# tj12323/GeoPurify

Hardware: AMD Instinct MI355X
Metric: scenes/sec (ScanNet-val shape) + pooled-feature GB/s vs HBM peak (higher is better)
Workload: dtype f32 (student convolutions and pooling: f16 hi/lo split operands, 3 MFMAs per product, fp32 accumulate)

## Files before the change

geopurify_amd/_lib.py:

```python
import ctypes
import os
from ctypes import POINTER, c_char_p, c_double, c_float, c_int32, c_int64, c_size_t, c_uint32, c_uint64, c_void_p

_HERE = os.path.dirname(os.path.abspath(__file__))
LIB_PATH = os.environ.get("GP_LIB") or os.path.join(_HERE, "libgeopurify_hip.so")

_P = c_void_p
GP_KNN_MAX_K = 127
GP_KNN_QUERY_MAX_K = 32
GP_ELEM_F32, GP_ELEM_F16, GP_ELEM_BF16 = 0, 1, 2
GP_LABEL_U8, GP_LABEL_I16, GP_LABEL_I32, GP_LABEL_I64 = 0, 1, 2, 3

SIGNATURES = {
    "gp_version": (c_int32, []),
    "gp_last_error": (c_char_p, []),
    "gp_debug_set": (c_int32, [c_int32, c_int32]),
    "gp_debug_ptr": (c_int32, [c_int32, _P, c_size_t]),
    "gp_voxelize_workspace_bytes": (c_size_t, [c_int64]),
    "gp_voxelize_f64": (c_int32, [_P, c_int64, POINTER(c_double), _P, _P, _P, _P, _P, _P, _P, c_size_t, _P]),
    "gp_fnv_hash_f64": (c_int32, [_P, c_int64, _P, _P]),
    "gp_project_points_f64": (c_int32, [_P, c_int64, POINTER(c_double), c_double, c_double, c_double,
                                        c_double, _P, c_int32, c_int32, c_int32, c_double, _P, _P, _P]),
    "gp_render_depth_f64": (c_int32, [_P, c_int64, POINTER(c_double), c_double, c_double, c_double, c_double,
                                      c_int32, c_int32, c_int32, _P, _P]),
# ... 11 lines not shown
    "gp_quantize_batched_workspace_bytes": (c_size_t, [c_int64]),
    "gp_quantize_batched": (c_int32, [_P, c_int64, _P, _P, _P, _P, _P, _P, _P, c_size_t, _P]),
    "gp_segment_labels": (c_int32, [_P, c_int64, _P, _P, _P, c_int64, c_int64, c_int32, _P, _P]),
    "gp_sparse_conv": (c_int32, [_P, c_int64, _P, c_int64, _P, c_int32, c_int32, c_int32, _P, _P, _P,
                                 c_int64, c_int32, _P, c_int64, _P]),
    "gp_conv_pairs_workspace_bytes": (c_size_t, [c_int64, c_int32]),
    "gp_conv_pairs_build": (c_int32, [_P, c_int64, c_int32, c_int32, _P, _P, _P, _P, _P, _P, _P, c_size_t, _P]),
    "gp_conv_chunk_plan_workspace_bytes": (c_size_t, [c_int64, c_int32]),
    "gp_conv_chunk_plan": (c_int32, [_P, c_int64, c_int32, c_int32, c_int32, c_int32, c_int32, _P, _P, _P, c_size_t, _P]),
    "gp_conv_weights_split": (c_int32, [_P, c_int32, c_int32, c_int32, c_float, _P, _P, _P]),
    "gp_split_f16": (c_int32, [_P, c_int64, c_int32, c_int64, _P, _P, c_int64, _P]),
    "gp_sparse_conv_f16x3": (c_int32, [_P, c_int64, _P, _P, c_int64, _P, _P, _P, _P, _P, c_int32, c_int64, c_int64, c_int32, _P, _P,
                                       c_int32, c_int32, _P, _P, _P, _P, c_int64, c_int32, _P, c_int64, _P, _P,
                                       c_int64, c_int32, POINTER(c_int32), POINTER(c_int32), POINTER(c_int32), _P, _P,
                                       _P, _P, c_int64, _P, c_int32, c_int32, _P]),
    "gp_conv_weights_split_blocked": (c_int32, [_P, c_int32, c_int32, c_int32, c_float, _P, _P, c_int32, _P]),
    "gp_pow2_scale": (c_int32, [_P, c_int64, c_int32, c_int64, _P, _P, c_size_t, _P]),
    "gp_voxel_rows_operands": (c_int32, [_P, c_int64, c_int32, _P, c_int64, c_int32, _P, _P, c_int64, _P, _P, c_int64, c_int32, _P, c_int64,
                                         _P, _P, _P, c_size_t, _P]),
    "gp_split_f16_scaled": (c_int32, [_P, c_int64, c_int32, c_int64, _P, _P, c_int64, _P, _P, _P, _P]),
    "gp_rcb_order": (c_int32, [_P, c_int64, c_int32, c_int32, _P, _P, _P]),
    "gp_rows_renumber_i32": (c_int32, [_P, c_int64, c_int32, _P, _P, _P, _P]),
    "gp_l2norm_rows": (c_int32, [_P, c_int64, c_int32, c_int64, _P]),
    "gp_embed_head_f16x3": (c_int32, [_P, _P, c_int64, _P, _P, _P, c_int64, c_int32, c_int32, c_float, c_int32, _P, c_int64, _P, _P, c_float, _P, _P]),
    "gp_knn_workspace_bytes": (c_size_t, [c_int64]),
    "gp_knn_lattice": (c_int32, [_P, _P, _P, c_int64, c_int32, _P, _P, c_size_t, _P]),
    "gp_knn_lattice_two_pass": (c_int32, [_P, _P, _P, c_int64, c_int32, _P, _P, c_size_t, _P]),
    "gp_knn_batched_workspace_bytes": (c_size_t, [c_int64]),
    "gp_knn_batched": (c_int32, [_P, _P, c_int64, c_int32, _P, _P, _P, c_size_t, _P]),
    "gp_affinity_softmax": (c_int32, [_P, c_int64, c_int32, _P, c_int32, c_int64, c_float, _P, _P]),
# ... 232 lines not shown
```

geopurify_amd/csrc/sparse_conv_v2.hip:

```cpp
#include <cstring>
#include <type_traits>
#include <rocprim/device/device_scan.hpp>

#include <hip/hip_fp16.h>

#include <stdlib.h>

#include "gp_common.h"
#include "gp_gfx950.h"
#include "gp_scan_bytes.h"

namespace {

constexpr int TM = 256, TN = 256, TK = 32;
constexpr int NT2 = 512;
constexpr int APITCH = 32;
__device__ __forceinline__ int sw_slot(int row, int slot) {
    const int h = (0x78 >> (((row >> 2) & 3) * 2)) & 3;
    return slot ^ h;
}

__device__ __forceinline__ void pair_decode(int64_t i, int kv, const int32_t *__restrict__ R, int nchunks, int &c, int &k, int64_t &u) {
    const int row_q = (int)(i / kv);
    int lo = 0, hi = nchunks - 1;
// ... 22 lines not shown
__global__ void pair_emit_kernel(const int32_t *__restrict__ nm, const int32_t *__restrict__ sc, int64_t nv, int kv,
                                 const int32_t *__restrict__ R, int nchunks, int32_t *__restrict__ pair_in, int32_t *__restrict__ pair_pos,
                                 int32_t *__restrict__ seg_off ) {
    int64_t total = (int64_t)kv * nv;
    int64_t i = blockIdx.x * (int64_t)blockDim.x + threadIdx.x;
    if (i >= total) return;
    int c, k; int64_t u;
    pair_decode(i, kv, R, nchunks, c, k, u);
    u = u < 0 ? 0 : (u >= nv ? nv - 1 : u);
    int in = nm[(int64_t)k * nv + u];
    int s = sc[i];
    pair_pos[(int64_t)k * nv + u] = in >= 0 ? s : -1;
    if (in >= 0) pair_in[s] = in;
    if (u == (int64_t)R[c]) seg_off[c * kv + k] = s;
    if (i == total - 1) seg_off[(c + 1) * kv] = s + (in >= 0 ? 1 : 0);
}
__global__ void chunk_count_kernel(const int32_t *__restrict__ nm, int64_t nv, int kv, int granule, int32_t *__restrict__ cnt ) {
    const int g = blockIdx.x, k = blockIdx.y;
    const int64_t r0 = (int64_t)g * granule, r1 = r0 + granule < nv ? r0 + granule : nv;
    int c = 0;
    for (int64_t u = r0 + threadIdx.x; u < r1; u += blockDim.x) c += nm[(int64_t)k * nv + u] >= 0;
    c = gp_wave_sum(c);
    __shared__ int s_c[4];
    if (gp_lane() == 0) s_c[threadIdx.x >> 6] = c;
    __syncthreads();
    if (threadIdx.x == 0) cnt[g * 32 + k] = s_c[0] + s_c[1] + s_c[2] + s_c[3];
}
constexpr int CP_WIN = 512;
__device__ __forceinline__ int cp_sum32(int v) {
    v += __builtin_amdgcn_update_dpp(0, v, 0xB1, 0xF, 0xF, true);
// ... 735 lines not shown
__device__ __forceinline__ void q24_batch_decode(const u32x4 (&th)[NL], const u32x2 (&tl)[NL], const unsigned (&te)[NL], const unsigned (&tsel)[NL],
                                                 int cnt, unsigned q, bool act, float (&a)[8]) {
#pragma unroll
    for (int i = 0; i < NL; ++i)
        if (i < cnt && act) q24_row_decode(th[i], tl[i], __builtin_amdgcn_perm(0u, te[i], tsel[i] + q), a);
}

template <bool WIDE , bool NO_CENTRE = false ,
          int WALK = 0 >
__global__ void __launch_bounds__(256) __attribute__((amdgpu_waves_per_eu(WALK ? GP_P2_WAVES : 4, WALK ? GP_P2_WAVES : 4)))
conv_phase2_q24_kernel(const unsigned char *__restrict__ pb, int64_t e_off, const int32_t *__restrict__ pair_pos, int64_t nv,
                       int kv, int cout, const float *__restrict__ scale, const float *__restrict__ shift,
                       const float *__restrict__ residual, int64_t ld_res, int relu, float *__restrict__ y, int64_t ld_y,
                       _Float16 *__restrict__ y_hi, _Float16 *__restrict__ y_lo, int64_t ld_yh, int64_t row_begin, int64_t row_count,
                       int pair_base, float *__restrict__ y_inv_scale, const _Float16 *__restrict__ res_hi,
                       const _Float16 *__restrict__ res_lo, int64_t ld_rh, const float *__restrict__ res_inv, int plane_flags) {
    const bool y_il = (plane_flags & 2) != 0, r_il = (plane_flags & 4) != 0;
    const int lane = gp_lane();
    const int64_t wave0 = (blockIdx.x * (int64_t)blockDim.x + threadIdx.x) >> 6, n_waves = ((int64_t)gridDim.x * blockDim.x) >> 6;
    const int64_t row_end = (row_begin + row_count < nv) ? row_begin + row_count : nv;
    int64_t u = row_begin + wave0;
    if (u >= row_end) return;
    const bool rowscale = y_inv_scale && y_hi && cout <= 1024;
    const int kv_read = NO_CENTRE ? (kv >> 1) : -1;
    int mypos_next = (lane < kv && lane != kv_read) ? pair_pos[(int64_t)lane * nv + u] : -1;
    float sc0[8], sh0[8];
    {
        const int c = lane * 8;
#pragma unroll
        for (int h = 0; h < 2; ++h) {
            const float4 a = (scale && c < cout) ? *reinterpret_cast<const float4 *>(scale + c + h * 4) : make_float4(1.f, 1.f, 1.f, 1.f);
            const float4 b = (shift && c < cout) ? *reinterpret_cast<const float4 *>(shift + c + h * 4) : make_float4(0.f, 0.f, 0.f, 0.f);
            sc0[h * 4] = a.x; sc0[h * 4 + 1] = a.y; sc0[h * 4 + 2] = a.z; sc0[h * 4 + 3] = a.w;
            sh0[h * 4] = b.x; sh0[h * 4 + 1] = b.y; sh0[h * 4 + 2] = b.z; sh0[h * 4 + 3] = b.w;
        }
    }
    if constexpr (WALK != 0) {
        static_assert(!WIDE && !NO_CENTRE, "the pipelined walk is for cout = 256 and 512");
        constexpr int NQ = 2 * WALK, NL = GP_P2_NL;
        const int c = lane * 8;
        const bool act = c < NQ * 128;
        const unsigned q = (unsigned)c >> 7, f = ((unsigned)c >> 3) & 15u;
        const unsigned off16 = q * 384u + f * 16u, off8 = q * 384u + 256u + f * 8u;
        const unsigned char *pb_e = pb + e_off;
        const unsigned long long kvmask = (kv >= 64) ? ~0ull : ((1ull << kv) - 1ull);
        auto load_pos = [&](int64_t r) { return (lane < kv && r < row_end) ? pair_pos[(int64_t)lane * nv + r] : -1; };
        auto wait_all = [] { __builtin_amdgcn_s_waitcnt(0x0f70); };
        u32x4 thA[NL], thB[NL];
        u32x2 tlA[NL], tlB[NL];
        unsigned teA[NL], teB[NL], tselA[NL], tselB[NL];
        int cntA, cntB;
        int posA = mypos_next, posB = load_pos(u + n_waves);
        unsigned long long mA = __ballot(posA >= 0) & kvmask;
        q24_batch_issue<NL, NQ>(thA, tlA, teA, tselA, cntA, pb, pb_e, posA, mA, off16, off8, act, pair_base);
        wait_all();
        unsigned long long mB = __ballot(posB >= 0) & kvmask;
        q24_batch_issue<NL, NQ>(thB, tlB, teB, tselB, cntB, pb, pb_e, posB, mB, off16, off8, act, pair_base);
        int pos2 = load_pos(u + 2 * n_waves);
        auto row = [&](u32x4 (&th)[NL], u32x2 (&tl)[NL], unsigned (&te)[NL], unsigned (&tsel)[NL], int &cnt, int &posX, unsigned long long &mX) __attribute__((always_inline)) {
            u32x4 r0 = {0u, 0u, 0u, 0u}, r1 = {0u, 0u, 0u, 0u};
            float ri = 1.f;
            if (act) {
                if (residual) {
                    r0 = *reinterpret_cast<const u32x4 *>(residual + u * ld_res + c);
                    r1 = *reinterpret_cast<const u32x4 *>(residual + u * ld_res + c + 4);
                } else if (res_hi) {
                    const _Float16 *rph = r_il ? res_hi + u * ld_rh + ((c >> 5) << 6) + (c & 31) : res_hi + u * ld_rh + c;
                    const _Float16 *rpl = r_il ? rph + 32 : res_lo + u * ld_rh + c;
                    r0 = *reinterpret_cast<const u32x4 *>(rph);
                    r1 = *reinterpret_cast<const u32x4 *>(rpl);
                    if (res_inv) ri = res_inv[u];
                }
            }
            float a[8];
#pragma unroll
            for (int j = 0; j < 8; ++j) a[j] = 0.f;
            q24_batch_decode<NL>(th, tl, te, tsel, cnt, q, act, a);
            while (mX) {
                q24_batch_issue<NL, NQ>(th, tl, te, tsel, cnt, pb, pb_e, posX, mX, off16, off8, act, pair_base);
                q24_batch_decode<NL>(th, tl, te, tsel, cnt, q, act, a);
            }
            wait_all();
            float amax = 0.f;
// ... 2 lines not shown
                for (int j = 0; j < 8; ++j) a[j] = a[j] * sc0[j] + sh0[j];
                if (residual) {
#pragma unroll
                    for (int j = 0; j < 4; ++j) { a[j] += __uint_as_float(r0[j]); a[j + 4] += __uint_as_float(r1[j]); }
                }
                if (res_hi) {
                    const f16x8 rh = __builtin_bit_cast(f16x8, r0), rl = __builtin_bit_cast(f16x8, r1);
#pragma unroll
                    for (int j = 0; j < 8; ++j) a[j] += ((float)rh[j] + (float)rl[j]) * ri;
                }
                if (relu) {
#pragma unroll
                    for (int j = 0; j < 8; ++j) a[j] = fmaxf(a[j], 0.f);
                }
                if (y) {
                    *reinterpret_cast<float4 *>(y + u * ld_y + c) = make_float4(a[0], a[1], a[2], a[3]);
                    *reinterpret_cast<float4 *>(y + u * ld_y + c + 4) = make_float4(a[4], a[5], a[6], a[7]);
                }
#pragma unroll
                for (int j = 0; j < 8; ++j) amax = fmaxf(amax, fabsf(a[j]));
            }
            float s = 1.f;
            if (rowscale) {
                amax = gp_wave_max(amax);
                s = gp_pow2_for(amax);
                if (lane == 0) y_inv_scale[u] = 1.f / s;
            }
            if (y_hi && act) {
                f16x8 h, l;
#pragma unroll
                for (int j = 0; j < 8; ++j) gp_split_f16(a[j] * s, h, l, j);
                _Float16 *ph = y_il ? y_hi + u * ld_yh + ((c >> 5) << 6) + (c & 31) : y_hi + u * ld_yh + c;
                _Float16 *pl = y_il ? ph + 32 : y_lo + u * ld_yh + c;
                *reinterpret_cast<f16x8 *>(ph) = h;
                *reinterpret_cast<f16x8 *>(pl) = l;
            }
            posX = pos2;
            mX = __ballot(posX >= 0) & kvmask;
            q24_batch_issue<NL, NQ>(th, tl, te, tsel, cnt, pb, pb_e, posX, mX, off16, off8, act, pair_base);
            pos2 = load_pos(u + 3 * n_waves);
        };
        for (;;) {
            row(thA, tlA, teA, tselA, cntA, posA, mA);
            u += n_waves;
            if (u >= row_end) break;
            row(thB, tlB, teB, tselB, cntB, posB, mB);
            u += n_waves;
            if (u >= row_end) break;
// ... 216 lines not shown
    size_t tb = gp_scan_bytes<int32_t>(total);
    char *tmp = cv.take<char>(tb);
    if (!cv.ok()) { gp_set_error("gp_conv_pairs_build: workspace too small (%zu < %zu)", workspace_bytes, cv.off); return GP_ENOMEM; }
    hipStream_t s = gp_stream(stream_);
    int blocks = (int)((total + 255) / 256);
    int nseg = num_chunks * kv;
    pair_flags_kernel<<<blocks, 256, 0, s>>>(nbr_map, nv, kv, chunk_row_off, num_chunks, f);
    GP_CHECK_HIP(rocprim::exclusive_scan(tmp, tb, f, sc, (int32_t)0, (size_t)total, rocprim::plus<int32_t>(), s));
    pair_emit_kernel<<<blocks, 256, 0, s>>>(nbr_map, sc, nv, kv, chunk_row_off, num_chunks, pair_in, pair_pos, seg_off);
    tile_start_kernel<<<1, 64, 0, s>>>(seg_off, nseg, tile_start);
    tile_desc_kernel<<<(nseg + 255) / 256, 256, 0, s>>>(seg_off, tile_start, nseg, kv, reinterpret_cast<int4 *>(tile_desc));
    GP_CHECK_LAUNCH();
    return GP_OK;
}

extern "C" size_t gp_conv_chunk_plan_workspace_bytes(int64_t nv, int32_t granule_rows) {
    if (nv <= 0 || granule_rows <= 0) return 0;
    return (size_t)((nv + granule_rows - 1) / granule_rows) * 32 * sizeof(int32_t);
}
extern "C" int gp_conv_chunk_plan(const int32_t *nbr_map, int64_t nv, int32_t kv, int32_t granule_rows, int32_t col_tiles,
                                  int32_t target_tiles, int32_t max_chunks, int32_t *chunk_row_off, int32_t *n_chunks, void *workspace,
                                  size_t workspace_bytes, void *stream_) {
    GP_CHECK_ARG(nbr_map && chunk_row_off && n_chunks && workspace && nv > 0 && kv > 0 && kv <= 32, "gp_conv_chunk_plan: null/empty argument");
    GP_CHECK_ARG(granule_rows >= 64 && granule_rows <= 65535 && col_tiles >= 1 && target_tiles >= col_tiles && max_chunks >= 1, "gp_conv_chunk_plan: bad sizes");
    const int64_t ngran = (nv + granule_rows - 1) / granule_rows;
    GP_CHECK_ARG(workspace_bytes >= gp_conv_chunk_plan_workspace_bytes(nv, granule_rows), "gp_conv_chunk_plan: workspace too small");
    hipStream_t s = gp_stream(stream_);
    int32_t *cnt = static_cast<int32_t *>(workspace);
    chunk_count_kernel<<<dim3((unsigned)ngran, (unsigned)kv), 256, 0, s>>>(nbr_map, nv, kv, granule_rows, cnt);
    chunk_plan_kernel<<<1, 256, 0, s>>>(cnt, (int)ngran, kv, granule_rows, nv, col_tiles, target_tiles, max_chunks, chunk_row_off, n_chunks);
// ... 41 lines not shown
    return GP_OK;
}

extern "C" int gp_split_f16_scaled(const float *x, int64_t ld_x, int32_t d, int64_t n, void *hi, void *lo, int64_t ld_h,
                                   const float *scale, float *row_inv_scale, const int32_t *dst_row, void *stream_) {
    GP_CHECK_ARG(x && hi && n > 0 && d > 0 && d % 4 == 0 && ld_x % 4 == 0 && ld_h % 4 == 0, "gp_split_f16_scaled: bad argument");
    GP_CHECK_ARG(lo || (d % 32 == 0 && ld_h >= 2 * (int64_t)d), "gp_split_f16_scaled: lo = NULL asks for interleaved rows in hi: d %% 32 == 0 and ld_h >= 2 d");
    GP_CHECK_ARG(!(scale && row_inv_scale), "gp_split_f16_scaled: one global scale OR per-row scales");
    int64_t waves = n < 16384 ? n : 16384;
    split_rows_scaled_kernel<<<(unsigned)((waves * 64 + 255) / 256), 256, 0, gp_stream(stream_)>>>(
        x, ld_x, d, n, static_cast<_Float16 *>(hi), static_cast<_Float16 *>(lo), ld_h, scale, row_inv_scale, dst_row);
    GP_CHECK_LAUNCH();
    return GP_OK;
}

extern "C" int gp_sparse_conv_f16x3(const float *x, int64_t ld_x, const void *x_hi, const void *x_lo, int64_t ld_xh,
                                    const int32_t *pair_in, const int32_t *pair_pos,
                                    const int32_t *pair_off, const int32_t *tile_start, const int32_t *tile_desc,
                                    int32_t nseg, int64_t num_pairs, int64_t nv, int32_t kv,
                                    const void *w_hi, const void *w_lo, int32_t cin, int32_t cout, float *partial,
                                    const float *scale, const float *shift, const float *residual, int64_t ld_res,
                                    int32_t relu, float *y, int64_t ld_y, void *y_hi, void *y_lo, int64_t ld_yh,
                                    int32_t num_chunks, const int32_t *chunk_row_off_host, const int32_t *chunk_tile_off_host,
                                    const int32_t *chunk_pair_off_host, const float *x_row_inv_scale, float *y_row_inv_scale,
                                    const void *res_hi, const void *res_lo, int64_t ld_rh, const float *res_row_inv_scale, int32_t w_blocked,
                                    int32_t plane_flags, void *stream_) {
    GP_CHECK_ARG(plane_flags >= 0 && plane_flags < 64, "gp_sparse_conv_f16x3: plane_flags is a mask of 1 (x interleaved), 2 (y interleaved), 4 (residual interleaved), 8 (fp32 partial rows), 16 (one dense offset: phase 1 writes y), 32 (phase 2 walks one row at a time)");
    const bool direct = (plane_flags & 16) != 0;
    GP_CHECK_ARG(!direct || (kv == 1 && num_pairs == nv && x_hi && y && ld_y == cout && !scale && !shift && !residual && !res_hi && !relu && !y_hi &&
                             !y_row_inv_scale && !(g_gp_knobs[3] & 16)),
                 "gp_sparse_conv_f16x3: plane_flags bit 4 is for kv = 1 with a pair for every row, pre-split x, contiguous fp32 y and no epilogue");
    GP_CHECK_ARG(!(plane_flags & 1) || (x_hi && ld_xh % 64 == 0 && cin % 32 == 0), "gp_sparse_conv_f16x3: interleaved x rows come as ONE tensor (x_hi) of 2 x cin halfs per row");
    GP_CHECK_ARG(!(plane_flags & 2) || (y_hi && ld_yh % 64 == 0 && (uintptr_t)y_hi % 16 == 0), "gp_sparse_conv_f16x3: interleaved y rows go to ONE tensor (y_hi) of 2 x cout halfs per row");
    GP_CHECK_ARG(!(plane_flags & 4) || (res_hi && ld_rh % 64 == 0), "gp_sparse_conv_f16x3: interleaved residual rows come as ONE tensor (res_hi)");
    GP_CHECK_ARG(w_blocked == 0 || w_blocked == 1, "gp_sparse_conv_f16x3: w_blocked is 0 (row-major weights) or 1 (gp_conv_weights_split_blocked)");
    GP_CHECK_ARG(!res_hi || ((res_lo || (plane_flags & 4)) && !residual && ld_rh % 8 == 0 && (uintptr_t)res_hi % 16 == 0 && (uintptr_t)res_lo % 16 == 0),
                 "gp_sparse_conv_f16x3: the residual comes as fp32 rows OR as 16-byte aligned split planes (res_hi + res_lo), not both");
    GP_CHECK_ARG(res_hi || (!res_lo && !res_row_inv_scale), "gp_sparse_conv_f16x3: res_lo / res_row_inv_scale belong to res_hi");
    GP_CHECK_ARG((x || (x_hi && (x_lo || (plane_flags & 1)))) && pair_in && pair_pos && pair_off && tile_start && tile_desc && nseg > 0 && w_hi && w_lo && partial && (y || y_hi), "gp_sparse_conv_f16x3: null argument");
    GP_CHECK_ARG(!x_hi || (ld_xh % 8 == 0 && (uintptr_t)x_hi % 16 == 0 && (uintptr_t)x_lo % 16 == 0), "gp_sparse_conv_f16x3: pre-split rows must be 16-byte aligned");
    GP_CHECK_ARG(!(plane_flags & 1) || !(g_gp_knobs[3] & 16), "gp_sparse_conv_f16x3: interleaved x rows need the LDS-DMA path");
// ... 63 lines not shown
                if (tune) conv_phase1_kernel<true><<<(unsigned)nblocks, NT2, sizeof(V2Smem), s>>>(P1R_ARGS);
                else conv_phase1_kernel<false><<<(unsigned)nblocks, NT2, sizeof(V2Smem), s>>>(P1R_ARGS);
#undef P1R_ARGS
            }
#undef P1_ARGS
        }
        if (direct) continue;
        const int64_t p2_full = (row_count * 64 + 255) / 256;
        int64_t p2_res = (int64_t)gp_cu_count() * p2_wg_per_cu;
        if (q24 && p2_wg_per_cu == 6) p2_res = (int64_t)gp_cu_count() * 4;
        const bool p2_pipe = q24 && cout <= 512 && !(plane_flags & 32) && !(g_conv_ablate & 256);
        if (p2_pipe) p2_res = (int64_t)gp_cu_count() * GP_P2_WAVES;
        const unsigned p2_grid = (unsigned)((p2_res > 0 && p2_res < p2_full) ? p2_res : p2_full);
#define P2Q_ARGS reinterpret_cast<const unsigned char *>(partial), q_e_off, pair_pos, nv, kv, cout, scale, shift, residual, ld_res, \
                 relu, y, ld_y, static_cast<_Float16 *>(y_hi), static_cast<_Float16 *>(y_lo), ld_yh, row_begin, row_count, pair_base, y_row_inv_scale, \
                 static_cast<const _Float16 *>(res_hi), static_cast<const _Float16 *>(res_lo), ld_rh, res_row_inv_scale, plane_flags
        if (p2_pipe && cout == 512) conv_phase2_q24_kernel<false, false, 2><<<p2_grid, 256, 0, s>>>(P2Q_ARGS);
        else if (p2_pipe) conv_phase2_q24_kernel<false, false, 1><<<p2_grid, 256, 0, s>>>(P2Q_ARGS);
        else if (q24 && cout <= 512 && (g_conv_ablate & 256)) conv_phase2_q24_kernel<false, true><<<p2_grid, 256, 0, s>>>(P2Q_ARGS);
        else if (q24 && cout > 512) conv_phase2_q24_kernel<true><<<p2_grid, 256, 0, s>>>(P2Q_ARGS);
        else if (q24) conv_phase2_q24_kernel<false><<<p2_grid, 256, 0, s>>>(P2Q_ARGS);
#undef P2Q_ARGS
        else
            conv_phase2_kernel<<<p2_grid, 256, 0, s>>>(
                partial, pair_pos, nv, kv, cout, scale, shift, residual, ld_res, relu, y, ld_y, static_cast<_Float16 *>(y_hi),
                static_cast<_Float16 *>(y_lo), ld_yh, row_begin, row_count, pair_base, y_row_inv_scale,
                static_cast<const _Float16 *>(res_hi), static_cast<const _Float16 *>(res_lo), ld_rh, res_row_inv_scale, plane_flags);
    }
    GP_CHECK_LAUNCH();
    return GP_OK;
}
```

geopurify_amd/ops.py:

```python
import ctypes

import numpy as np
import torch

from . import _lib
from ._lib import check


def _ptr(t):
    return ctypes.c_void_p(t.data_ptr()) if t is not None else None


def _stream():
    return ctypes.c_void_p(torch.cuda.current_stream().cuda_stream)


def _ws(nbytes, device):
    return torch.empty(max(int(nbytes), 256), dtype=torch.uint8, device=device)


def _chk(t, dtype, name):
    if t.dtype != dtype or not t.is_cuda or not t.is_contiguous():
        raise ValueError(f"{name}: expected contiguous CUDA {dtype}, got {t.dtype} cuda={t.is_cuda} contig={t.is_contiguous()}")
    return t
# ... 273 lines not shown
        kv, cin, cout = w.shape
    else:
        kv, (cin, cout) = 1, w.shape
    _chk(w, torch.float32, "w")
    if out is None:
        out = torch.empty((nv, cout), dtype=torch.float32, device=x.device)
    check(lib.gp_sparse_conv(_ptr(x), x.stride(0), _ptr(nbr_map) if kv > 1 else None, nv, _ptr(w), int(kv),
                             int(cin), int(cout), _ptr(scale), _ptr(shift), _ptr(residual),
                             residual.stride(0) if residual is not None else 0, int(bool(relu)), _ptr(out),
                             out.stride(0), _stream()), "gp_sparse_conv")
    return out


class ConvPairs:

    def __init__(self, pair_in, pair_pos, seg_off, tile_start, nseg, num_pairs, nv):
        self.pair_in, self.pair_pos, self.pair_off, self.tile_start = pair_in, pair_pos, seg_off, tile_start
        self.nseg, self.num_pairs, self.nv = nseg, num_pairs, nv
        self.partial = None
        self.num_chunks, self.chunk_row_off, self.chunk_tile_off, self.chunk_pair_off = 0, None, None, None

    def _set_chunks(self, rows, tiles, pairs):
        n = len(rows) - 1
        self.num_chunks = n
        self.chunk_row_off = (ctypes.c_int32 * (n + 1))(*rows)
        self.chunk_tile_off = (ctypes.c_int32 * (n + 1))(*tiles)
        self.chunk_pair_off = (ctypes.c_int32 * (n + 1))(*pairs)
        self.max_chunk_pairs = max(pairs[i + 1] - pairs[i] for i in range(n))

    def regroup(self, g):
        g = max(1, min(int(g), max(self.num_chunks, 1)))
        cp = ConvPairs(self.pair_in, self.pair_pos, self.pair_off, self.tile_start, self.nseg, self.num_pairs, self.nv)
        cp.tile_desc = self.tile_desc
        n = self.num_chunks
        idx = list(range(0, n, g)) + [n]
        ro, po, to = list(self.chunk_row_off), list(self.chunk_pair_off), list(self.chunk_tile_off)
        cp._set_chunks([ro[i] for i in idx], [to[i] for i in idx], [po[i] for i in idx])
        return cp


CONV_TARGET_TILES = None


def conv_pairs_build(nbr_map, chunk_rows="balanced", col_tiles=2):
    lib = _lib.load()
    kv, nv = nbr_map.shape
    dev = nbr_map.device
# ... 16 lines not shown
        ch = nv if chunk_rows is None else max(int(chunk_rows), 256)
        rows = list(range(0, nv, ch)) + [nv]
        nchunks = len(rows) - 1
        row_off = torch.tensor(rows, dtype=torch.int32, device=dev)
    nseg = nchunks * kv
    ws = _ws(lib.gp_conv_pairs_workspace_bytes(nv, kv), dev)
    pair_in = torch.empty(kv * nv, dtype=torch.int32, device=dev)
    pair_pos = torch.empty((kv, nv), dtype=torch.int32, device=dev)
    seg_off = torch.empty(nseg + 1, dtype=torch.int32, device=dev)
    tile_start = torch.empty(nseg + 1, dtype=torch.int32, device=dev)
    tile_desc = torch.empty(((kv * nv) // 256 + nseg + 1, 4), dtype=torch.int32, device=dev)
    check(lib.gp_conv_pairs_build(_ptr(nbr_map), nv, kv, nchunks, _ptr(row_off), _ptr(pair_in), _ptr(pair_pos), _ptr(seg_off),
                                  _ptr(tile_start), _ptr(tile_desc), _ptr(ws), ws.numel(), _stream()), "gp_conv_pairs_build")
    bounds = readback(torch.stack([seg_off[::kv], tile_start[::kv]]))
    num_pairs = bounds[0][-1]
    cp = ConvPairs(pair_in, pair_pos, seg_off, tile_start, nseg, num_pairs, nv)
    cp.tile_desc = tile_desc
    cp._set_chunks(rows, bounds[1], bounds[0])
    return cp


def conv_weights_split(w, scale_pow2, blocked=None, transpose_flip=False):
    lib = _lib.load()
    kv, cin, cout = w.shape
    if transpose_flip:
        if cout % 32 == 0 and cin % 256 == 0 and blocked is not False:
            hi = torch.empty((kv, cin // 256, cout // 32, 256, 32), dtype=torch.float16, device=w.device)
            lo = torch.empty_like(hi)
            check(lib.gp_conv_weights_split_blocked(_ptr(w), kv, cout, cin, float(scale_pow2), _ptr(hi), _ptr(lo), 1, _stream()),
                  "gp_conv_weights_split_blocked")
            return hi, lo
        return conv_weights_split(w.flip(0).transpose(1, 2).contiguous(), scale_pow2, blocked)
    if blocked is None:
        blocked = cin % 32 == 0 and cout % 256 == 0
# ... 82 lines not shown
    w_blocked = int(w_hi.dim() == 5)
    nv = pairs.nv
    dev = w_hi.device
    if dense_single_offset:
        partial = torch.empty(64, dtype=torch.float32, device=dev)
    else:
        if pairs.partial is None or pairs.partial.shape[1] < cout or pairs.partial.shape[0] < max(pairs.max_chunk_pairs, 1):
            pairs.partial = torch.empty((max(pairs.max_chunk_pairs, 1), cout), dtype=torch.float32, device=dev)
        partial = pairs.partial
    if out is None and (want_f32 or out_split is None):
        out = torch.empty((nv, cout), dtype=torch.float32, device=dev)
    xh, xl = x_split if x_split is not None else (None, None)
    yh, yl = out_split if out_split is not None else (None, None)
    plane_flags = (1 if (xh is not None and xl is None) else 0) | (2 if (yh is not None and yl is None) else 0) | \
                  (4 if (rh is not None and rl is None) else 0) | (8 if fp32_partials else 0) | (16 if dense_single_offset else 0) | (32 if reference_walk else 0)
    check(lib.gp_sparse_conv_f16x3(_ptr(x), x.stride(0) if x is not None else 0, _ptr(xh), _ptr(xl),
                                   xh.stride(0) if xh is not None else 0, _ptr(pairs.pair_in), _ptr(pairs.pair_pos),
                                   _ptr(pairs.pair_off), _ptr(pairs.tile_start), _ptr(pairs.tile_desc), pairs.nseg, pairs.num_pairs, nv, kv, _ptr(w_hi), _ptr(w_lo), cin, cout,
                                   _ptr(partial), _ptr(scale), _ptr(shift), _ptr(residual),
                                   residual.stride(0) if residual is not None else 0, int(bool(relu)), _ptr(out),
                                   out.stride(0) if out is not None else 0, _ptr(yh), _ptr(yl), yh.stride(0) if yh is not None else 0,
                                   int(pairs.num_chunks), pairs.chunk_row_off, pairs.chunk_tile_off, pairs.chunk_pair_off,
                                   _ptr(x_row_inv), _ptr(out_row_inv), _ptr(rh), _ptr(rl), rh.stride(0) if rh is not None else 0, _ptr(ri),
                                   w_blocked, plane_flags, _stream()),
          "gp_sparse_conv_f16x3")
    return out


def interleave_planes(hi, lo):
    n, c = hi.shape
    return torch.stack([hi.reshape(n, c // 32, 32), lo.reshape(n, c // 32, 32)], dim=2).reshape(n, 2 * c).contiguous()


def deinterleave_planes(t):
    n, c2 = t.shape
    v = t.reshape(n, c2 // 64, 2, 32)
    return v[:, :, 0].reshape(n, c2 // 2).contiguous(), v[:, :, 1].reshape(n, c2 // 2).contiguous()


# ... 2010 lines not shown
```

include/geopurify_hip.h:

```cpp
#ifndef GEOPURIFY_HIP_H
#define GEOPURIFY_HIP_H

#include <stddef.h>
#include <stdint.h>

#ifdef __cplusplus
extern "C" {
#endif

#define GP_OK 0
#define GP_EINVAL (-22)
#define GP_ENOMEM (-12)
#define GP_EHIP (-5)
#define GP_ERANGE (-34)

#define GP_KNN_MAX_K 127

#define GP_ELEM_F32 0
#define GP_ELEM_F16 1
#define GP_ELEM_BF16 2

int gp_version(void);
int gp_debug_set(int32_t key, int32_t value);
int gp_debug_ptr(int32_t key, void *device_buffer, size_t bytes);
// ... 66 lines not shown
int gp_voxel_rows_operands(const float *f, int64_t ld_f, int32_t d, const float *geo, int64_t ld_geo, int32_t dg,
                           const int64_t *order, const int64_t *seg_start, int64_t nv, const int32_t *row_map, float *x,
                           int64_t ld_x, int32_t cin_pad, void *rows, int64_t ld_rows, float *row_inv_scale, float *scale2,
                           void *workspace, size_t workspace_bytes, void *stream);
int gp_sparse_conv_f16x3(const float *x, int64_t ld_x, const void *x_hi, const void *x_lo, int64_t ld_xh,
                         const int32_t *pair_in, const int32_t *pair_pos,
                         const int32_t *seg_off, const int32_t *tile_start, const int32_t *tile_desc,
                         int32_t nseg, int64_t num_pairs, int64_t nv, int32_t kv,
                         const void *w_hi, const void *w_lo, int32_t cin, int32_t cout, float *partial,
                         const float *scale, const float *shift, const float *residual, int64_t ld_res,
                         int32_t relu, float *y, int64_t ld_y, void *y_hi, void *y_lo, int64_t ld_yh,
                         int32_t num_chunks, const int32_t *chunk_row_off_host, const int32_t *chunk_tile_off_host,
                         const int32_t *chunk_pair_off_host, const float *x_row_inv_scale, float *y_row_inv_scale,
                         const void *res_hi, const void *res_lo, int64_t ld_rh, const float *res_row_inv_scale, int32_t w_blocked,
                         int32_t plane_flags, void *stream);
int gp_conv_weights_split_blocked(const float *w, int32_t kv, int32_t cin, int32_t cout, float scale_pow2,
                                  void *w_hi, void *w_lo, int32_t transpose_flip, void *stream);
int gp_l2norm_rows(float *x, int64_t ld, int32_t d, int64_t n, void *stream);
int gp_embed_head_f16x3(const void *x_hi, const void *x_lo, int64_t ld_x, const float *x_row_inv_scale, const void *w_hi,
                        const void *w_lo, int64_t nv, int32_t cin, int32_t cout, float out_scale, int32_t l2_normalize,
                        float *y, int64_t ld_y, void *e_hi, void *e_lo, float plane_scale,
                        const int32_t *e_dst_row ,
                        void *stream);

int gp_rcb_order(const int32_t *coords, int64_t nv, int32_t chunk_rows, int32_t leaf_rows, int32_t *sigma, int32_t *rho, void *stream);
int gp_rows_renumber_i32(const int32_t *nbr, int64_t nv, int32_t k, const int32_t *sigma, const int32_t *rho, int32_t *out,
                         void *stream);

size_t gp_knn_workspace_bytes(int64_t nv);
int gp_knn_lattice(const void *grid, const int32_t *coords, const int32_t *ids, int64_t nv,
// ... 417 lines not shown
```

Before: 46.97.

## Transpose pair positions to row-major for coalesced phase-2 walk loads

Adds a kernel that transposes the offset-major pair_pos map into a row-major [nv,32] table once per pair build, and the pipelined phase-2 conv walk reads a row's 32 positions contiguously instead of striding by nv. It also routes residual, output and split-plane addresses through an opaque lane offset so the compiler can use a scalar base plus a vector offset, and it seeds the first row directly. This costs an extra transpose kernel and a buffer of nv*32 int32 per pair set, in exchange for fewer scattered loads in the walk.

Measured after the change: 46.90. No clear change (-0.2%).

```diff
diff --git a/geopurify_amd/_lib.py b/geopurify_amd/_lib.py
--- a/geopurify_amd/_lib.py
+++ b/geopurify_amd/_lib.py
@@ -49,6 +49,11 @@
                                        c_int32, c_int32, _P, _P, _P, _P, c_int64, c_int32, _P, c_int64, _P, _P,
                                        c_int64, c_int32, POINTER(c_int32), POINTER(c_int32), POINTER(c_int32), _P, _P,
                                        _P, _P, c_int64, _P, c_int32, c_int32, _P]),
+    "gp_conv_pair_rows": (c_int32, [_P, c_int64, c_int32, _P, _P]),
+    "gp_sparse_conv_f16x3_rows": (c_int32, [_P, c_int64, _P, _P, c_int64, _P, _P, _P, _P, _P, c_int32, c_int64, c_int64, c_int32, _P, _P,
+                                            c_int32, c_int32, _P, _P, _P, _P, c_int64, c_int32, _P, c_int64, _P, _P,
+                                            c_int64, c_int32, POINTER(c_int32), POINTER(c_int32), POINTER(c_int32), _P, _P,
+                                            _P, _P, c_int64, _P, c_int32, c_int32, _P, _P]),
     "gp_conv_weights_split_blocked": (c_int32, [_P, c_int32, c_int32, c_int32, c_float, _P, _P, c_int32, _P]),
     "gp_pow2_scale": (c_int32, [_P, c_int64, c_int32, c_int64, _P, _P, c_size_t, _P]),
     "gp_voxel_rows_operands": (c_int32, [_P, c_int64, c_int32, _P, c_int64, c_int32, _P, _P, c_int64, _P, _P, c_int64, c_int32, _P, c_int64,
diff --git a/geopurify_amd/csrc/sparse_conv_v2.hip b/geopurify_amd/csrc/sparse_conv_v2.hip
--- a/geopurify_amd/csrc/sparse_conv_v2.hip
+++ b/geopurify_amd/csrc/sparse_conv_v2.hip
@@ -60,6 +60,16 @@
     if (in >= 0) pair_in[s] = in;
     if (u == (int64_t)R[c]) seg_off[c * kv + k] = s;
     if (i == total - 1) seg_off[(c + 1) * kv] = s + (in >= 0 ? 1 : 0);
+}
+__global__ void __launch_bounds__(256)
+pair_rows_kernel(const int32_t *__restrict__ pair_pos, int64_t nv, int kv, int32_t *__restrict__ pos_rows) {
+    __shared__ int32_t s_t[64][33];
+    const int64_t u0 = (int64_t)blockIdx.x * 64;
+    const int tid = threadIdx.x, r = tid & 63;
+    for (int k = tid >> 6; k < 32; k += 4) s_t[r][k] = (k < kv && u0 + r < nv) ? pair_pos[(int64_t)k * nv + u0 + r] : -1;
+    __syncthreads();
+    const int64_t rows = nv - u0 < 64 ? nv - u0 : 64;
+    for (int i = tid; i < rows * 32; i += 256) pos_rows[u0 * 32 + i] = s_t[i >> 5][i & 31];
 }
 __global__ void chunk_count_kernel(const int32_t *__restrict__ nm, int64_t nv, int kv, int granule, int32_t *__restrict__ cnt ) {
     const int g = blockIdx.x, k = blockIdx.y;
@@ -825,7 +835,8 @@
                        const float *__restrict__ residual, int64_t ld_res, int relu, float *__restrict__ y, int64_t ld_y,
                        _Float16 *__restrict__ y_hi, _Float16 *__restrict__ y_lo, int64_t ld_yh, int64_t row_begin, int64_t row_count,
                        int pair_base, float *__restrict__ y_inv_scale, const _Float16 *__restrict__ res_hi,
-                       const _Float16 *__restrict__ res_lo, int64_t ld_rh, const float *__restrict__ res_inv, int plane_flags) {
+                       const _Float16 *__restrict__ res_lo, int64_t ld_rh, const float *__restrict__ res_inv, int plane_flags,
+                       const int32_t *__restrict__ pos_rows) {
     const bool y_il = (plane_flags & 2) != 0, r_il = (plane_flags & 4) != 0;
     const int lane = gp_lane();
     const int64_t wave0 = (blockIdx.x * (int64_t)blockDim.x + threadIdx.x) >> 6, n_waves = ((int64_t)gridDim.x * blockDim.x) >> 6;
@@ -849,19 +860,28 @@
     if constexpr (WALK != 0) {
         static_assert(!WIDE && !NO_CENTRE, "the pipelined walk is for cout = 256 and 512");
         constexpr int NQ = 2 * WALK, NL = GP_P2_NL;
+        u = row_begin + blockIdx.x * (int64_t)(blockDim.x >> 6) + __builtin_amdgcn_readfirstlane((int)(threadIdx.x >> 6));
         const int c = lane * 8;
         const bool act = c < NQ * 128;
         const unsigned q = (unsigned)c >> 7, f = ((unsigned)c >> 3) & 15u;
         const unsigned off16 = q * 384u + f * 16u, off8 = q * 384u + 256u + f * 8u;
         const unsigned char *pb_e = pb + e_off;
         const unsigned long long kvmask = (kv >= 64) ? ~0ull : ((1ull << kv) - 1ull);
-        auto load_pos = [&](int64_t r) { return (lane < kv && r < row_end) ? pair_pos[(int64_t)lane * nv + r] : -1; };
+        auto lane_at = [](const void *row, unsigned off) {
+            asm volatile("" : "+v"(off));
+            return const_cast<char *>(static_cast<const char *>(row)) + off;
+        };
+        auto load_pos = [&](int64_t r) {
+            if (pos_rows) return (lane < 32 && r < row_end) ? *reinterpret_cast<const int32_t *>(lane_at(pos_rows + r * 32, lane * 4u)) : -1;
+            return (lane < kv && r < row_end) ? pair_pos[(int64_t)lane * nv + r] : -1;
+        };
         auto wait_all = [] { __builtin_amdgcn_s_waitcnt(0x0f70); };
+        const unsigned c_il = ((c >> 5) << 6) + (c & 31);
         u32x4 thA[NL], thB[NL];
         u32x2 tlA[NL], tlB[NL];
         unsigned teA[NL], teB[NL], tselA[NL], tselB[NL];
         int cntA, cntB;
-        int posA = mypos_next, posB = load_pos(u + n_waves);
+        int posA = load_pos(u), posB = load_pos(u + n_waves);
         unsigned long long mA = __ballot(posA >= 0) & kvmask;
         q24_batch_issue<NL, NQ>(thA, tlA, teA, tselA, cntA, pb, pb_e, posA, mA, off16, off8, act, pair_base);
         wait_all();
@@ -873,11 +893,12 @@
             float ri = 1.f;
             if (act) {
                 if (residual) {
-                    r0 = *reinterpret_cast<const u32x4 *>(residual + u * ld_res + c);
-                    r1 = *reinterpret_cast<const u32x4 *>(residual + u * ld_res + c + 4);
+                    const char *rp = lane_at(residual + u * ld_res, c * 4u);
+                    r0 = *reinterpret_cast<const u32x4 *>(rp);
+                    r1 = *reinterpret_cast<const u32x4 *>(rp + 16);
                 } else if (res_hi) {
-                    const _Float16 *rph = r_il ? res_hi + u * ld_rh + ((c >> 5) << 6) + (c & 31) : res_hi + u * ld_rh + c;
-                    const _Float16 *rpl = r_il ? rph + 32 : res_lo + u * ld_rh + c;
+                    const char *rph = lane_at(res_hi + u * ld_rh, r_il ? c_il * 2u : c * 2u);
+                    const char *rpl = r_il ? rph + 64 : lane_at(res_lo + u * ld_rh, c * 2u);
                     r0 = *reinterpret_cast<const u32x4 *>(rph);
                     r1 = *reinterpret_cast<const u32x4 *>(rpl);
                     if (res_inv) ri = res_inv[u];
@@ -910,8 +931,9 @@
                     for (int j = 0; j < 8; ++j) a[j] = fmaxf(a[j], 0.f);
                 }
                 if (y) {
-                    *reinterpret_cast<float4 *>(y + u * ld_y + c) = make_float4(a[0], a[1], a[2], a[3]);
-                    *reinterpret_cast<float4 *>(y + u * ld_y + c + 4) = make_float4(a[4], a[5], a[6], a[7]);
+                    char *yp = lane_at(y + u * ld_y, c * 4u);
+                    *reinterpret_cast<float4 *>(yp) = make_float4(a[0], a[1], a[2], a[3]);
+                    *reinterpret_cast<float4 *>(yp + 16) = make_float4(a[4], a[5], a[6], a[7]);
                 }
 #pragma unroll
                 for (int j = 0; j < 8; ++j) amax = fmaxf(amax, fabsf(a[j]));
@@ -926,8 +948,8 @@
                 f16x8 h, l;
 #pragma unroll
                 for (int j = 0; j < 8; ++j) gp_split_f16(a[j] * s, h, l, j);
-                _Float16 *ph = y_il ? y_hi + u * ld_yh + ((c >> 5) << 6) + (c & 31) : y_hi + u * ld_yh + c;
-                _Float16 *pl = y_il ? ph + 32 : y_lo + u * ld_yh + c;
+                char *ph = lane_at(y_hi + u * ld_yh, y_il ? c_il * 2u : c * 2u);
+                char *pl = y_il ? ph + 64 : lane_at(y_lo + u * ld_yh, c * 2u);
                 *reinterpret_cast<f16x8 *>(ph) = h;
                 *reinterpret_cast<f16x8 *>(pl) = l;
             }
@@ -1174,6 +1196,14 @@
     return GP_OK;
 }
 
+extern "C" int gp_conv_pair_rows(const int32_t *pair_pos, int64_t nv, int32_t kv, int32_t *pos_rows, void *stream_) {
+    GP_CHECK_ARG(pair_pos && pos_rows && nv > 0 && kv > 0 && kv <= 32, "gp_conv_pair_rows: null/empty argument, or kv > 32");
+    GP_CHECK_ARG(nv < (1ll << 31) / 32, "gp_conv_pair_rows: kernel map too large");
+    pair_rows_kernel<<<(unsigned)((nv + 63) / 64), 256, 0, gp_stream(stream_)>>>(pair_pos, nv, kv, pos_rows);
+    GP_CHECK_LAUNCH();
+    return GP_OK;
+}
+
 extern "C" size_t gp_conv_chunk_plan_workspace_bytes(int64_t nv, int32_t granule_rows) {
     if (nv <= 0 || granule_rows <= 0) return 0;
     return (size_t)((nv + granule_rows - 1) / granule_rows) * 32 * sizeof(int32_t);
@@ -1245,17 +1275,17 @@
     return GP_OK;
 }
 
-extern "C" int gp_sparse_conv_f16x3(const float *x, int64_t ld_x, const void *x_hi, const void *x_lo, int64_t ld_xh,
-                                    const int32_t *pair_in, const int32_t *pair_pos,
-                                    const int32_t *pair_off, const int32_t *tile_start, const int32_t *tile_desc,
-                                    int32_t nseg, int64_t num_pairs, int64_t nv, int32_t kv,
-                                    const void *w_hi, const void *w_lo, int32_t cin, int32_t cout, float *partial,
-                                    const float *scale, const float *shift, const float *residual, int64_t ld_res,
-                                    int32_t relu, float *y, int64_t ld_y, void *y_hi, void *y_lo, int64_t ld_yh,
-                                    int32_t num_chunks, const int32_t *chunk_row_off_host, const int32_t *chunk_tile_off_host,
-                                    const int32_t *chunk_pair_off_host, const float *x_row_inv_scale, float *y_row_inv_scale,
-                                    const void *res_hi, const void *res_lo, int64_t ld_rh, const float *res_row_inv_scale, int32_t w_blocked,
-                                    int32_t plane_flags, void *stream_) {
+extern "C" int gp_sparse_conv_f16x3_rows(const float *x, int64_t ld_x, const void *x_hi, const void *x_lo, int64_t ld_xh,
+                                         const int32_t *pair_in, const int32_t *pair_pos,
+                                         const int32_t *pair_off, const int32_t *tile_start, const int32_t *tile_desc,
+                                         int32_t nseg, int64_t num_pairs, int64_t nv, int32_t kv,
+                                         const void *w_hi, const void *w_lo, int32_t cin, int32_t cout, float *partial,
+                                         const float *scale, const float *shift, const float *residual, int64_t ld_res,
+                                         int32_t relu, float *y, int64_t ld_y, void *y_hi, void *y_lo, int64_t ld_yh,
+                                         int32_t num_chunks, const int32_t *chunk_row_off_host, const int32_t *chunk_tile_off_host,
+                                         const int32_t *chunk_pair_off_host, const float *x_row_inv_scale, float *y_row_inv_scale,
+                                         const void *res_hi, const void *res_lo, int64_t ld_rh, const float *res_row_inv_scale, int32_t w_blocked,
+                                         int32_t plane_flags, const int32_t *pos_rows, void *stream_) {
     GP_CHECK_ARG(plane_flags >= 0 && plane_flags < 64, "gp_sparse_conv_f16x3: plane_flags is a mask of 1 (x interleaved), 2 (y interleaved), 4 (residual interleaved), 8 (fp32 partial rows), 16 (one dense offset: phase 1 writes y), 32 (phase 2 walks one row at a time)");
     const bool direct = (plane_flags & 16) != 0;
     GP_CHECK_ARG(!direct || (kv == 1 && num_pairs == nv && x_hi && y && ld_y == cout && !scale && !shift && !residual && !res_hi && !relu && !y_hi &&
@@ -1349,7 +1379,7 @@
         const unsigned p2_grid = (unsigned)((p2_res > 0 && p2_res < p2_full) ? p2_res : p2_full);
 #define P2Q_ARGS reinterpret_cast<const unsigned char *>(partial), q_e_off, pair_pos, nv, kv, cout, scale, shift, residual, ld_res, \
                  relu, y, ld_y, static_cast<_Float16 *>(y_hi), static_cast<_Float16 *>(y_lo), ld_yh, row_begin, row_count, pair_base, y_row_inv_scale, \
-                 static_cast<const _Float16 *>(res_hi), static_cast<const _Float16 *>(res_lo), ld_rh, res_row_inv_scale, plane_flags
+                 static_cast<const _Float16 *>(res_hi), static_cast<const _Float16 *>(res_lo), ld_rh, res_row_inv_scale, plane_flags, pos_rows
         if (p2_pipe && cout == 512) conv_phase2_q24_kernel<false, false, 2><<<p2_grid, 256, 0, s>>>(P2Q_ARGS);
         else if (p2_pipe) conv_phase2_q24_kernel<false, false, 1><<<p2_grid, 256, 0, s>>>(P2Q_ARGS);
         else if (q24 && cout <= 512 && (g_conv_ablate & 256)) conv_phase2_q24_kernel<false, true><<<p2_grid, 256, 0, s>>>(P2Q_ARGS);
@@ -1365,3 +1395,20 @@
     GP_CHECK_LAUNCH();
     return GP_OK;
 }
+
+extern "C" int gp_sparse_conv_f16x3(const float *x, int64_t ld_x, const void *x_hi, const void *x_lo, int64_t ld_xh,
+                                    const int32_t *pair_in, const int32_t *pair_pos,
+                                    const int32_t *pair_off, const int32_t *tile_start, const int32_t *tile_desc,
+                                    int32_t nseg, int64_t num_pairs, int64_t nv, int32_t kv,
+                                    const void *w_hi, const void *w_lo, int32_t cin, int32_t cout, float *partial,
+                                    const float *scale, const float *shift, const float *residual, int64_t ld_res,
+                                    int32_t relu, float *y, int64_t ld_y, void *y_hi, void *y_lo, int64_t ld_yh,
+                                    int32_t num_chunks, const int32_t *chunk_row_off_host, const int32_t *chunk_tile_off_host,
+                                    const int32_t *chunk_pair_off_host, const float *x_row_inv_scale, float *y_row_inv_scale,
+                                    const void *res_hi, const void *res_lo, int64_t ld_rh, const float *res_row_inv_scale, int32_t w_blocked,
+                                    int32_t plane_flags, void *stream_) {
+    return gp_sparse_conv_f16x3_rows(x, ld_x, x_hi, x_lo, ld_xh, pair_in, pair_pos, pair_off, tile_start, tile_desc, nseg, num_pairs, nv, kv, w_hi,
+                                     w_lo, cin, cout, partial, scale, shift, residual, ld_res, relu, y, ld_y, y_hi, y_lo, ld_yh, num_chunks,
+                                     chunk_row_off_host, chunk_tile_off_host, chunk_pair_off_host, x_row_inv_scale, y_row_inv_scale, res_hi,
+                                     res_lo, ld_rh, res_row_inv_scale, w_blocked, plane_flags, nullptr, stream_);
+}
diff --git a/geopurify_amd/ops.py b/geopurify_amd/ops.py
--- a/geopurify_amd/ops.py
+++ b/geopurify_amd/ops.py
@@ -311,8 +311,9 @@
 
 class ConvPairs:
 
-    def __init__(self, pair_in, pair_pos, seg_off, tile_start, nseg, num_pairs, nv):
+    def __init__(self, pair_in, pair_pos, seg_off, tile_start, nseg, num_pairs, nv, pos_rows=None):
         self.pair_in, self.pair_pos, self.pair_off, self.tile_start = pair_in, pair_pos, seg_off, tile_start
+        self.pos_rows = pos_rows
         self.nseg, self.num_pairs, self.nv = nseg, num_pairs, nv
         self.partial = None
         self.num_chunks, self.chunk_row_off, self.chunk_tile_off, self.chunk_pair_off = 0, None, None, None
@@ -327,7 +328,7 @@
 
     def regroup(self, g):
         g = max(1, min(int(g), max(self.num_chunks, 1)))
-        cp = ConvPairs(self.pair_in, self.pair_pos, self.pair_off, self.tile_start, self.nseg, self.num_pairs, self.nv)
+        cp = ConvPairs(self.pair_in, self.pair_pos, self.pair_off, self.tile_start, self.nseg, self.num_pairs, self.nv, self.pos_rows)
         cp.tile_desc = self.tile_desc
         n = self.num_chunks
         idx = list(range(0, n, g)) + [n]
@@ -374,10 +375,19 @@
                                   _ptr(tile_start), _ptr(tile_desc), _ptr(ws), ws.numel(), _stream()), "gp_conv_pairs_build")
     bounds = readback(torch.stack([seg_off[::kv], tile_start[::kv]]))
     num_pairs = bounds[0][-1]
-    cp = ConvPairs(pair_in, pair_pos, seg_off, tile_start, nseg, num_pairs, nv)
+    cp = ConvPairs(pair_in, pair_pos, seg_off, tile_start, nseg, num_pairs, nv, conv_pair_rows(pair_pos) if kv <= 32 else None)
     cp.tile_desc = tile_desc
     cp._set_chunks(rows, bounds[1], bounds[0])
     return cp
+
+
+def conv_pair_rows(pair_pos):
+    lib = _lib.load()
+    _chk(pair_pos, torch.int32, "pair_pos")
+    kv, nv = pair_pos.shape
+    pos_rows = torch.empty((nv, 32), dtype=torch.int32, device=pair_pos.device)
+    check(lib.gp_conv_pair_rows(_ptr(pair_pos), nv, kv, _ptr(pos_rows), _stream()), "gp_conv_pair_rows")
+    return pos_rows
 
 
 def conv_weights_split(w, scale_pow2, blocked=None, transpose_flip=False):
@@ -490,7 +500,8 @@
     yh, yl = out_split if out_split is not None else (None, None)
     plane_flags = (1 if (xh is not None and xl is None) else 0) | (2 if (yh is not None and yl is None) else 0) | \
                   (4 if (rh is not None and rl is None) else 0) | (8 if fp32_partials else 0) | (16 if dense_single_offset else 0) | (32 if reference_walk else 0)
-    check(lib.gp_sparse_conv_f16x3(_ptr(x), x.stride(0) if x is not None else 0, _ptr(xh), _ptr(xl),
+    pos_rows = None if (reference_walk or fp32_partials) else pairs.pos_rows
+    check(lib.gp_sparse_conv_f16x3_rows(_ptr(x), x.stride(0) if x is not None else 0, _ptr(xh), _ptr(xl),
                                    xh.stride(0) if xh is not None else 0, _ptr(pairs.pair_in), _ptr(pairs.pair_pos),
                                    _ptr(pairs.pair_off), _ptr(pairs.tile_start), _ptr(pairs.tile_desc), pairs.nseg, pairs.num_pairs, nv, kv, _ptr(w_hi), _ptr(w_lo), cin, cout,
                                    _ptr(partial), _ptr(scale), _ptr(shift), _ptr(residual),
@@ -498,7 +509,7 @@
                                    out.stride(0) if out is not None else 0, _ptr(yh), _ptr(yl), yh.stride(0) if yh is not None else 0,
                                    int(pairs.num_chunks), pairs.chunk_row_off, pairs.chunk_tile_off, pairs.chunk_pair_off,
                                    _ptr(x_row_inv), _ptr(out_row_inv), _ptr(rh), _ptr(rl), rh.stride(0) if rh is not None else 0, _ptr(ri),
-                                   w_blocked, plane_flags, _stream()),
+                                   w_blocked, plane_flags, _ptr(pos_rows), _stream()),
           "gp_sparse_conv_f16x3")
     return out
 
diff --git a/include/geopurify_hip.h b/include/geopurify_hip.h
--- a/include/geopurify_hip.h
+++ b/include/geopurify_hip.h
@@ -104,6 +104,18 @@
                          const int32_t *chunk_pair_off_host, const float *x_row_inv_scale, float *y_row_inv_scale,
                          const void *res_hi, const void *res_lo, int64_t ld_rh, const float *res_row_inv_scale, int32_t w_blocked,
                          int32_t plane_flags, void *stream);
+int gp_conv_pair_rows(const int32_t *pair_pos, int64_t nv, int32_t kv, int32_t *pos_rows, void *stream);
+int gp_sparse_conv_f16x3_rows(const float *x, int64_t ld_x, const void *x_hi, const void *x_lo, int64_t ld_xh,
+                              const int32_t *pair_in, const int32_t *pair_pos,
+                              const int32_t *seg_off, const int32_t *tile_start, const int32_t *tile_desc,
+                              int32_t nseg, int64_t num_pairs, int64_t nv, int32_t kv,
+                              const void *w_hi, const void *w_lo, int32_t cin, int32_t cout, float *partial,
+                              const float *scale, const float *shift, const float *residual, int64_t ld_res,
+                              int32_t relu, float *y, int64_t ld_y, void *y_hi, void *y_lo, int64_t ld_yh,
+                              int32_t num_chunks, const int32_t *chunk_row_off_host, const int32_t *chunk_tile_off_host,
+                              const int32_t *chunk_pair_off_host, const float *x_row_inv_scale, float *y_row_inv_scale,
+                              const void *res_hi, const void *res_lo, int64_t ld_rh, const float *res_row_inv_scale, int32_t w_blocked,
+                              int32_t plane_flags, const int32_t *pos_rows, void *stream);
 int gp_conv_weights_split_blocked(const float *w, int32_t kv, int32_t cin, int32_t cout, float scale_pow2,
                                   void *w_hi, void *w_lo, int32_t transpose_flip, void *stream);
 int gp_l2norm_rows(float *x, int64_t ld, int32_t d, int64_t n, void *stream);
```
